# hzxie/RMNet

Measured on AMD Instinct MI355X. Metric: frames/sec at 480p, 1 object, T=5 memory; memory-read HBM GB/s vs peak, higher is better.
Workload: dtype f32 convs; memory read = fp16 operands (K, V, q, P rounded to 11 bits), fp32 accumulate (RMNET_BANK_F16): the frame loop's default for clips with one object -- on one-object 480x854 clips whose masks HAVE a boundary (tests/live_fixture.py) mask IoU vs the CPU path 0.99993-0.99997 and foreground logi

## Files before the change

include/rmnet_hip.h:

```cpp
#ifndef RMNET_HIP_H_
#define RMNET_HIP_H_

#include <stddef.h>
#include <stdint.h>

#ifdef __cplusplus
extern "C" {
#endif

#define RMNET_ABI_VERSION 6

enum {
  RMNET_OK = 0,
  RMNET_E_INVALID_ARG = -1,
  RMNET_E_WORKSPACE = -2,
  RMNET_E_LAUNCH = -3,
  RMNET_E_UNSUPPORTED = -4
};

int rmnet_abi_version(void);
const char *rmnet_error_string(int code);

size_t rmnet_region_map_workspace_bytes(int B, int K, int H, int W);
int rmnet_region_map_f32(const float *mask, int B, int K, int H, int W, float prob_threshold,
// ... 83 lines not shown

#define RMNET_CONV_RELU_IN 1
#define RMNET_CONV_RELU_OUT 2
int rmnet_conv3x3_split_f32(const float *x, const void *wpack, const float *w_unscale, const float *bias, const float *res, int flags,
                            int N, int H, int W, int Cin, float *out, int32_t *range_word, void *stream);

int rmnet_conv3x3_split_lds_f32(const float *x, const void *wpack, const float *w_unscale, const float *bias, const float *res,
                                int flags, int N, int H, int W, int Cin, float *out, int32_t *range_word, void *stream);

int rmnet_conv3x3_rows_f32(const float *x, const void *wpack, const float *w_unscale, const float *bias, const float *res, int flags,
                           int N, int H, int W, int Cin, float *out, int32_t *range_word, void *stream);

int rmnet_conv_split_f32(const float *x, const void *wpack, const float *w_unscale, const float *shift, const float *res, int flags,
                         int N, int H, int W, int Cin, int Cout, int ksize, int stride, float *out, float *out2, int out_split,
                         int32_t *range_word, void *stream);

#define RMNET_CONV_X_SPLIT 4
#define RMNET_CONV_OUT_SPLIT 8
int rmnet_conv_split_pre_f32(const void *x, const void *wpack, const float *w_unscale, const float *shift, const float *res, int flags,
                             int N, int H, int W, int Cin, int Cout, int ksize, int stride, void *out, float *out2, int out_split,
                             int32_t *range_word, void *stream);
int rmnet_split_act_f32(const float *x, long long M, int C, int relu, void *out, int32_t *range_word, void *stream);

int rmnet_conv_rows_pre_f32(const void *x, const void *wpack, const float *w_unscale, const float *shift, const float *res, int flags,
                            int N, int H, int W, int Cin, int Cout, int ksize, int stride, void *out, float *out2, int out_split,
                            int32_t *range_word, void *stream);

int rmnet_stem_split_f32(const float *frame, const float *mask, const float *other, const void *wpack, const float *w_unscale,
                         const float *shift, int N, int H, int W, float *out, int32_t *range_word, void *stream);

int rmnet_flow_stem_f32(const float *img0, const float *img1, long long batch_stride0, long long batch_stride1, const void *wpack,
                        const float *w_unscale, const float *bias, int N, int H, int W, int Hpad, int Wpad, int lh, int lw, float *out, int32_t *range_word, void *stream);

int rmnet_pred_head_f32(const float *x, const float *w, const float *bias, int n, int Hq, int Wq, int C, float *out, void *stream);

#define RMNET_FLOW_RELU 1
#define RMNET_FLOW_LEAKY 2
#define RMNET_FLOW_TRANSPOSED 4
int rmnet_flow_conv_f32(const float *x, int x_ld, const void *wpack, const float *w_unscale, const float *shift, int flags, int N, int H,
                        int W, int Cin, int Cout, int ksize, int stride, float *out, int out_ld, int coff, int32_t *range_word,
                        void *stream);

size_t rmnet_flow_head_workspace_bytes(int N, int H, int W, int Cin);
int rmnet_flow_head_f32(const float *x, int x_ld, const float *wpack, const float *bias, int N, int H, int W, int Cin, float *out,
                        void *workspace, size_t workspace_bytes, void *stream);

// ... 54 lines not shown
```

rmnet_amd/_lib.py:

```python

import ctypes
import os

_HERE = os.path.dirname(os.path.abspath(__file__))
LIB_PATH = os.environ.get('RMNET_HIP_LIB') or os.path.join(_HERE, 'librmnet_hip.so')

c_f32p = ctypes.c_void_p
c_i32p = ctypes.c_void_p
c_f64p = ctypes.POINTER(ctypes.c_double)
c_hostp = ctypes.c_void_p

SIGNATURES = {
    'rmnet_abi_version': (ctypes.c_int, []),
    'rmnet_error_string': (ctypes.c_char_p, [ctypes.c_int]),
    'rmnet_region_map_workspace_bytes': (ctypes.c_size_t, [ctypes.c_int] * 4),
    'rmnet_region_map_f32': (ctypes.c_int, [
        c_f32p, ctypes.c_int, ctypes.c_int, ctypes.c_int, ctypes.c_int, ctypes.c_float, ctypes.c_int,
        ctypes.c_int, c_f32p, c_i32p, c_i32p, ctypes.c_int, ctypes.c_int, ctypes.c_int, ctypes.c_int,
        ctypes.c_int, ctypes.c_void_p, ctypes.c_size_t, ctypes.c_void_p]),
    'rmnet_region_map_warped_f32': (ctypes.c_int, [
        c_f32p, c_f32p, ctypes.c_int, ctypes.c_int, ctypes.c_int, ctypes.c_int, ctypes.c_float, ctypes.c_int,
        ctypes.c_int, c_f32p, c_i32p, c_i32p, ctypes.c_int, ctypes.c_int, ctypes.c_int, ctypes.c_int,
        ctypes.c_int, c_f32p, ctypes.c_void_p, ctypes.c_size_t, ctypes.c_void_p]),
    'rmnet_boxes_to_cell_rects_i32': (ctypes.c_int, [
# ... 53 lines not shown
        c_f32p, c_f32p, c_f32p, c_f32p, c_f32p, c_f32p, ctypes.c_int, ctypes.c_longlong, ctypes.c_int, c_f32p, ctypes.c_void_p]),
    'rmnet_upsample2x_add_nhwc_f32': (ctypes.c_int, [
        c_f32p, c_f32p, ctypes.c_longlong, ctypes.c_int, ctypes.c_int, ctypes.c_int, c_f32p, ctypes.c_void_p]),
    'rmnet_affine_relu_maxpool_nhwc_f32': (ctypes.c_int, [
        c_f32p, c_f32p, c_f32p, ctypes.c_longlong, ctypes.c_int, ctypes.c_int, ctypes.c_int, c_f32p, ctypes.c_void_p]),
    'rmnet_conv3x3_split_f32': (ctypes.c_int, [
        c_f32p, ctypes.c_void_p, c_f32p, c_f32p, c_f32p, ctypes.c_int, ctypes.c_int, ctypes.c_int, ctypes.c_int, ctypes.c_int,
        c_f32p, c_i32p, ctypes.c_void_p]),
    'rmnet_conv3x3_split_lds_f32': (ctypes.c_int, [
        c_f32p, ctypes.c_void_p, c_f32p, c_f32p, c_f32p, ctypes.c_int, ctypes.c_int, ctypes.c_int, ctypes.c_int, ctypes.c_int,
        c_f32p, c_i32p, ctypes.c_void_p]),
    'rmnet_conv3x3_rows_f32': (ctypes.c_int, [
        c_f32p, ctypes.c_void_p, c_f32p, c_f32p, c_f32p, ctypes.c_int, ctypes.c_int, ctypes.c_int, ctypes.c_int, ctypes.c_int,
        c_f32p, c_i32p, ctypes.c_void_p]),
    'rmnet_conv_split_f32': (ctypes.c_int, [
        c_f32p, ctypes.c_void_p, c_f32p, c_f32p, c_f32p, ctypes.c_int, ctypes.c_int, ctypes.c_int, ctypes.c_int, ctypes.c_int,
        ctypes.c_int, ctypes.c_int, ctypes.c_int, c_f32p, c_f32p, ctypes.c_int, c_i32p, ctypes.c_void_p]),
    'rmnet_conv_split_pre_f32': (ctypes.c_int, [
        ctypes.c_void_p, ctypes.c_void_p, c_f32p, c_f32p, c_f32p, ctypes.c_int, ctypes.c_int, ctypes.c_int, ctypes.c_int, ctypes.c_int,
        ctypes.c_int, ctypes.c_int, ctypes.c_int, ctypes.c_void_p, c_f32p, ctypes.c_int, c_i32p, ctypes.c_void_p]),
    'rmnet_conv_rows_pre_f32': (ctypes.c_int, [
        ctypes.c_void_p, ctypes.c_void_p, c_f32p, c_f32p, c_f32p, ctypes.c_int, ctypes.c_int, ctypes.c_int, ctypes.c_int, ctypes.c_int,
        ctypes.c_int, ctypes.c_int, ctypes.c_int, ctypes.c_void_p, c_f32p, ctypes.c_int, c_i32p, ctypes.c_void_p]),
    'rmnet_split_act_f32': (ctypes.c_int, [
        c_f32p, ctypes.c_longlong, ctypes.c_int, ctypes.c_int, ctypes.c_void_p, c_i32p, ctypes.c_void_p]),
    'rmnet_stem_split_f32': (ctypes.c_int, [
        c_f32p, c_f32p, c_f32p, ctypes.c_void_p, c_f32p, c_f32p, ctypes.c_int, ctypes.c_int, ctypes.c_int, c_f32p, c_i32p,
        ctypes.c_void_p]),
    'rmnet_flow_stem_f32': (ctypes.c_int, [
        c_f32p, c_f32p, ctypes.c_longlong, ctypes.c_longlong, ctypes.c_void_p, c_f32p, c_f32p, ctypes.c_int, ctypes.c_int, ctypes.c_int,
        ctypes.c_int, ctypes.c_int, ctypes.c_int, ctypes.c_int, c_f32p, c_i32p, ctypes.c_void_p]),
    'rmnet_pred_head_f32': (ctypes.c_int, [
        c_f32p, c_f32p, c_f32p, ctypes.c_int, ctypes.c_int, ctypes.c_int, ctypes.c_int, c_f32p, ctypes.c_void_p]),
    'rmnet_flow_conv_f32': (ctypes.c_int, [
        c_f32p, ctypes.c_int, ctypes.c_void_p, c_f32p, c_f32p, ctypes.c_int, ctypes.c_int, ctypes.c_int, ctypes.c_int, ctypes.c_int,
        ctypes.c_int, ctypes.c_int, ctypes.c_int, c_f32p, ctypes.c_int, ctypes.c_int, c_i32p, ctypes.c_void_p]),
    'rmnet_flow_head_workspace_bytes': (ctypes.c_size_t, [ctypes.c_int] * 4),
    'rmnet_flow_head_f32': (ctypes.c_int, [
        c_f32p, ctypes.c_int, c_f32p, c_f32p, ctypes.c_int, ctypes.c_int, ctypes.c_int, ctypes.c_int, c_f32p, ctypes.c_void_p,
        ctypes.c_size_t, ctypes.c_void_p]),
    'rmnet_flow_up_f32': (ctypes.c_int, [
        c_f32p, c_f32p, ctypes.c_int, ctypes.c_int, ctypes.c_int, c_f32p, ctypes.c_int, ctypes.c_int, ctypes.c_void_p]),
    'rmnet_flow_affine_f32': (ctypes.c_int, [
        c_f32p, c_f32p, c_f32p, ctypes.c_int, ctypes.c_int, c_f32p, ctypes.c_void_p]),
    'rmnet_flow_affine_workspace_bytes': (ctypes.c_size_t, [ctypes.c_int, ctypes.c_int]),
    'rmnet_flow_affine_f32_host': (ctypes.c_int, [
# ... 72 lines not shown
```

rmnet_amd/csrc/conv_split.hip:

```cpp
#include "split_f16.h"

namespace rmnet {
namespace {

struct SplitArgs {
  const float* x;
  const _Float16* xs;
  const u32x4* wp;
  const float* unscale;
  const float* shift;
  const float* res;
  float* out;
  float* out2;
  _Float16* outs;
  int* range;
  int M, H, W, Ho, Wo, Cin, Cout, csplit, ksize, stride, pad, relu_in, relu_out;
};

template <int WM, int WN, int TI, int TJ, int WPE, bool XS, bool OS>
__global__ __launch_bounds__(kThreads) __attribute__((amdgpu_waves_per_eu(WPE))) void conv_split(SplitArgs a) {
  static_assert(WM * WN * 64 == kThreads, "8 waves");
  constexpr int MT = WM * TI * 16, NT = WN * TJ * 16;
  constexpr int XI = MT / 64;
  constexpr int WI = NT / 64;
  constexpr int kXPlane = MT * kKT, kWPlane = NT * kKT;
  constexpr int kBufHalves = 2 * kXPlane + 2 * kWPlane;
  static_assert(2 * kBufHalves * 2 <= kLdsBytesPerCU, "LDS budget");
  __shared__ __attribute__((aligned(16))) _Float16 lds[2 * kBufHalves];

  const int tid = threadIdx.x, lane = tid & 63, wave = tid >> 6;
  const int wm = wave % WM, wn = wave / WM;
  const int m0 = blockIdx.x * MT, n0 = blockIdx.y * NT;
  const int CB = a.Cin / kKT, steps = a.ksize * a.ksize * CB;
  const int HWo = a.Ho * a.Wo;

  const int c4 = tid & 7;
  int pbase[XI], ph[XI], pw[XI];
#pragma unroll
  for (int i = 0; i < XI; ++i) {
    const int m = m0 + (tid >> 3) + 64 * i;
    const int n = m / HWo, r = m - n * HWo;
    const int ho = r / a.Wo, wo = r - ho * a.Wo;
    ph[i] = m < a.M ? ho * a.stride - a.pad : -4;
    pw[i] = wo * a.stride - a.pad;
    pbase[i] = (n * a.H + ph[i]) * a.W + pw[i];
  }
  f32x4 xr[XI];
  u32x4 xq[XI];
  u32x4 wr[WI];
  int bad = 0;

  auto load_x = [&](int s) {
    const int tap = s / CB, cb = s - tap * CB;
    const int ky = tap / a.ksize, kx = tap - ky * a.ksize;
#pragma unroll
    for (int i = 0; i < XI; ++i) {
      const int h = ph[i] + ky, w = pw[i] + kx;
      const bool in = (unsigned)h < (unsigned)a.H && (unsigned)w < (unsigned)a.W;
      if constexpr (XS) {
        if (in) {
          const unsigned off = (unsigned)(pbase[i] + ky * a.W + kx) * (unsigned)(2 * a.Cin) + (unsigned)(cb * (2 * kKT) + 8 * c4);
          xq[i] = *reinterpret_cast<const u32x4*>(a.xs + off);
        } else {
          xq[i] = u32x4{0u, 0u, 0u, 0u};
        }
      } else {
        if (in) {
          const size_t off = (size_t)(pbase[i] + ky * a.W + kx) * a.Cin + cb * kKT + 4 * c4;
// ... 118 lines not shown
  };
  constexpr bool kInTurn = !XS && TI > TJ && WPE == 4 && WI > 1;
  for (int s = 0; s + 1 < steps; ++s) {
    _Float16* nxt = lds + ((s + 1) & 1) * kBufHalves;
    load_x(s + 1);
    if constexpr (!kInTurn) load_w(s + 1);
    __builtin_amdgcn_sched_barrier(0);
    mma(lds + (s & 1) * kBufHalves, [&] {
      if constexpr (kInTurn) {
        __builtin_amdgcn_sched_barrier(0);
        load_w(s + 1);
        store_x(s + 1, nxt);
        __builtin_amdgcn_sched_barrier(0);
      }
    });
    __builtin_amdgcn_sched_barrier(0);
    if constexpr (!kInTurn) store_x(s + 1, nxt);
    store_w(nxt);
    __syncthreads();
  }
  mma(lds + ((steps - 1) & 1) * kBufHalves, [] {});

  f32x4 r[TI][TJ];
  if (a.res) {
#pragma unroll
    for (int i = 0; i < TI; ++i) {
      const int m = m0 + wm * TI * 16 + i * 16 + fr;
#pragma unroll
      for (int j = 0; j < TJ; ++j) {
        const int co = n0 + wn * TJ * 16 + j * 16 + 4 * fc;
        r[i][j] = m < a.M ? *reinterpret_cast<const f32x4*>(a.res + (size_t)m * a.Cout + co) : f32x4{0.f, 0.f, 0.f, 0.f};
      }
    }
  }
#pragma unroll
  for (int j = 0; j < TJ; ++j) {
    const int co = n0 + wn * TJ * 16 + j * 16 + 4 * fc;
    const f32x4 us = *reinterpret_cast<const f32x4*>(a.unscale + co) * kActUnscale;
    const f32x4 b = a.shift ? *reinterpret_cast<const f32x4*>(a.shift + co) : f32x4{0.f, 0.f, 0.f, 0.f};
#pragma unroll
    for (int i = 0; i < TI; ++i) acc[i][j] = (acc[i][j] + accx[i][j]) * us + b;
  }
#pragma unroll
  for (int j = 0; j < TJ; ++j)
#pragma unroll
    for (int i = 0; i < TI; ++i) asm volatile("" : "+v"(acc[i][j]));
#pragma unroll
  for (int j = 0; j < TJ; ++j) {
    const int co = n0 + wn * TJ * 16 + j * 16 + 4 * fc;
#pragma unroll
    for (int i = 0; i < TI; ++i) {
      const int m = m0 + wm * TI * 16 + i * 16 + fr;
      if (m >= a.M) continue;
      f32x4 v = acc[i][j];
      if (a.res) v += r[i][j];
      if (a.relu_out) {
#pragma unroll
        for (int e = 0; e < 4; ++e) v[e] = v[e] < 0.0f ? 0.0f : v[e];
      }
      if constexpr (OS) {
        half4 hi, lo;
        split4(v, hi, lo, bad);
        _Float16* o = a.outs + (size_t)m * (2 * a.Cout) + (co >> 5) * (2 * kKT) + (co & 31);
        *reinterpret_cast<half4*>(o) = hi;
        *reinterpret_cast<half4*>(o + kKT) = lo;
      } else {
        const size_t off = (size_t)m * a.Cout + co;
        if (!a.out2)
          *reinterpret_cast<f32x4*>(a.out + off) = v;
        else if (co < a.csplit)
          *reinterpret_cast<f32x4*>(a.out + (size_t)m * a.csplit + co) = v;
        else
          *reinterpret_cast<f32x4*>(a.out2 + (size_t)m * (a.Cout - a.csplit) + (co - a.csplit)) = v;
      }
    }
  }
  if (a.range && bad) atomicAdd(a.range, bad);
}

template <int WM, int WN, int TI, int TJ, int WPE, bool XS, bool OS>
void launch(const SplitArgs& a, hipStream_t st) {
  constexpr int MT = WM * TI * 16, NT = WN * TJ * 16;
  hipLaunchKernelGGL((conv_split<WM, WN, TI, TJ, WPE, XS, OS>), dim3((unsigned)((a.M + MT - 1) / MT), (unsigned)(a.Cout / NT)),
                     dim3(kThreads), 0, st, a);
}

template <bool XS, bool OS>
void launch_tile(const SplitArgs& a, hipStream_t st) {
  if (a.Cout % 256 == 0 && (long long)((a.M + 127) / 128) * (a.Cout / 256) >= 512)
    launch<2, 4, 4, 4, 2, XS, OS>(a, st);
  else if (a.Cout % 128 == 0)
    launch<2, 4, 4, 2, 4, XS, OS>(a, st);
  else
    launch<4, 2, 2, 2, 4, XS, OS>(a, st);
}

constexpr int kSplitActThreads = 256;
__global__ __launch_bounds__(kSplitActThreads) void split_act(const float* __restrict__ x, _Float16* __restrict__ out, size_t items,
                                                              int relu, int* range) {
  int bad = 0;
  for (size_t q = (size_t)blockIdx.x * kSplitActThreads + threadIdx.x; q < items; q += (size_t)gridDim.x * kSplitActThreads) {
    f32x4 v[2];
    v[0] = *reinterpret_cast<const f32x4*>(x + q * 8);
// ... 2 lines not shown
#pragma unroll
    for (int k = 0; k < 2; ++k) {
      if (relu) {
#pragma unroll
        for (int e = 0; e < 4; ++e) v[k][e] = v[k][e] < 0.0f ? 0.0f : v[k][e];
      }
      half4 h4, l4;
      split4(v[k], h4, l4, bad);
#pragma unroll
      for (int e = 0; e < 4; ++e) {
        hi[4 * k + e] = h4[e];
        lo[4 * k + e] = l4[e];
      }
    }
    _Float16* o = out + (q >> 2) * (2 * kKT) + (q & 3) * 8;
    *reinterpret_cast<half8*>(o) = hi;
    *reinterpret_cast<half8*>(o + kKT) = lo;
  }
  if (range && bad) atomicAdd(range, bad);
}

int conv_split_entry(const void* x, const void* wpack, const float* w_unscale, const float* shift, const float* res, int flags, int allowed,
                     int N, int H, int W, int Cin, int Cout, int ksize, int stride, void* out, float* out2, int out_split,
                     int32_t* range_word, void* stream) {
  if (!x || !wpack || !w_unscale || !out || N <= 0 || H <= 0 || W <= 0 || Cin <= 0 || Cout <= 0) return RMNET_E_INVALID_ARG;
  if (flags & ~allowed) return RMNET_E_INVALID_ARG;
  const bool xs = (flags & RMNET_CONV_X_SPLIT) != 0, os = (flags & RMNET_CONV_OUT_SPLIT) != 0;
  if (xs && (flags & RMNET_CONV_RELU_IN)) return RMNET_E_INVALID_ARG;
  if (os && out2) return RMNET_E_INVALID_ARG;
  if ((reinterpret_cast<uintptr_t>(x) | reinterpret_cast<uintptr_t>(wpack) | reinterpret_cast<uintptr_t>(w_unscale) |
       reinterpret_cast<uintptr_t>(shift) | reinterpret_cast<uintptr_t>(res) | reinterpret_cast<uintptr_t>(out) |
       reinterpret_cast<uintptr_t>(out2)) & 15)
    return RMNET_E_INVALID_ARG;
  if (out2 && (res || out_split <= 0 || out_split >= Cout || out_split % 4)) return RMNET_E_INVALID_ARG;
  if ((ksize != 1 && ksize != 3) || (stride != 1 && stride != 2)) return RMNET_E_UNSUPPORTED;
  if (Cin % kKT || Cout % 64) return RMNET_E_UNSUPPORTED;
  const int pad = ksize / 2;
  const int Ho = (H + 2 * pad - ksize) / stride + 1, Wo = (W + 2 * pad - ksize) / stride + 1;
  const long long Mi = (long long)N * H * W, M = (long long)N * Ho * Wo;
  if (Mi * Cin >= (1LL << 31) || M * Cout >= (1LL << 31)) return RMNET_E_UNSUPPORTED;
  const long long xbytes = Mi * Cin * 4, c1 = out2 ? out_split : Cout;
  if (overlap(out, M * c1 * 4, x, xbytes)) return RMNET_E_INVALID_ARG;
  if (os && res && overlap(out, M * c1 * 4, res, M * Cout * 4)) return RMNET_E_INVALID_ARG;
  if (out2) {
    if (overlap(out2, M * (Cout - c1) * 4, x, xbytes) || overlap(out2, M * (Cout - c1) * 4, out, M * c1 * 4)) return RMNET_E_INVALID_ARG;
  }
  SplitArgs a;
  a.x = xs ? nullptr : reinterpret_cast<const float*>(x);
  a.xs = xs ? reinterpret_cast<const _Float16*>(x) : nullptr;
  a.wp = reinterpret_cast<const u32x4*>(wpack); a.unscale = w_unscale; a.shift = shift; a.res = res;
  a.out = os ? nullptr : reinterpret_cast<float*>(out); a.out2 = out2; a.outs = os ? reinterpret_cast<_Float16*>(out) : nullptr;
  a.range = range_word; a.M = (int)M; a.H = H; a.W = W; a.Ho = Ho; a.Wo = Wo; a.Cin = Cin; a.Cout = Cout; a.csplit = (int)c1;
  a.ksize = ksize; a.stride = stride; a.pad = pad;
  a.relu_in = (flags & RMNET_CONV_RELU_IN) != 0;
  a.relu_out = (flags & RMNET_CONV_RELU_OUT) != 0;
  hipStream_t st = (hipStream_t)stream;
  if (xs && os) launch_tile<true, true>(a, st);
  else if (xs) launch_tile<true, false>(a, st);
  else if (os) launch_tile<false, true>(a, st);
  else launch_tile<false, false>(a, st);
  return check_launch();
}

}
}

extern "C" int rmnet_conv_split_f32(const float* x, const void* wpack, const float* w_unscale, const float* shift,
                                    const float* res, int flags, int N, int H, int W, int Cin, int Cout, int ksize, int stride,
                                    float* out, float* out2, int out_split, int32_t* range_word, void* stream) {
  return rmnet::conv_split_entry(x, wpack, w_unscale, shift, res, flags, RMNET_CONV_RELU_IN | RMNET_CONV_RELU_OUT, N, H, W, Cin, Cout,
                                 ksize, stride, out, out2, out_split, range_word, stream);
}

extern "C" int rmnet_conv_split_pre_f32(const void* x, const void* wpack, const float* w_unscale, const float* shift, const float* res,
                                        int flags, int N, int H, int W, int Cin, int Cout, int ksize, int stride, void* out, float* out2,
                                        int out_split, int32_t* range_word, void* stream) {
  return rmnet::conv_split_entry(x, wpack, w_unscale, shift, res, flags,
                                 RMNET_CONV_RELU_IN | RMNET_CONV_RELU_OUT | RMNET_CONV_X_SPLIT | RMNET_CONV_OUT_SPLIT, N, H, W, Cin, Cout,
                                 ksize, stride, out, out2, out_split, range_word, stream);
}

extern "C" int rmnet_split_act_f32(const float* x, long long M, int C, int relu, void* out, int32_t* range_word, void* stream) {
  using namespace rmnet;
  if (!x || !out || M <= 0 || C <= 0) return RMNET_E_INVALID_ARG;
  if ((reinterpret_cast<uintptr_t>(x) | reinterpret_cast<uintptr_t>(out)) & 15) return RMNET_E_INVALID_ARG;
  if (C % kKT) return RMNET_E_UNSUPPORTED;
  if (M > (1LL << 40) / C) return RMNET_E_UNSUPPORTED;
  if (overlap(out, M * C * 4, x, M * C * 4)) return RMNET_E_INVALID_ARG;
  const size_t items = (size_t)M * C / 8;
  const size_t blocks = (items + kSplitActThreads - 1) / kSplitActThreads;
  const unsigned grid = (unsigned)(blocks < (size_t)kNumCUs * 8 ? blocks : (size_t)kNumCUs * 8);
  hipLaunchKernelGGL(split_act, dim3(grid), dim3(kSplitActThreads), 0, (hipStream_t)stream, x, reinterpret_cast<_Float16*>(out), items,
                     relu != 0, range_word);
  return check_launch();
}
```

rmnet_amd/networks.py:

```python

import torch
import torch.nn.functional as F
from torch import nn


class _Bottleneck(nn.Module):

    def __init__(self, c_in, width, stride, project):
        super().__init__()
        c_out = width * 4
        self.conv1 = nn.Conv2d(c_in, width, 1, bias=False)
        self.bn1 = nn.BatchNorm2d(width)
        self.conv2 = nn.Conv2d(width, width, 3, stride=stride, padding=1, bias=False)
        self.bn2 = nn.BatchNorm2d(width)
        self.conv3 = nn.Conv2d(width, c_out, 1, bias=False)
        self.bn3 = nn.BatchNorm2d(c_out)
        self.relu = nn.ReLU(inplace=True)
        self.downsample = None
        if project:
            self.downsample = nn.Sequential(nn.Conv2d(c_in, c_out, 1, stride=stride, bias=False),
                                            nn.BatchNorm2d(c_out))

    def forward(self, x):
        if getattr(self, '_fused', False) and not self.training and x.is_cuda:
# ... 258 lines not shown


def set_split_conv_(module, enable):
    prev = {}
    for m in module.modules():
        if isinstance(m, (_Bottleneck, KeyValue, ResBlock, Refine, Decoder, EncoderMemory, EncoderQuery)):
            prev[m] = getattr(m, '_conv_split', False)
            m._conv_split = bool(enable) and getattr(m, '_wu', getattr(m, '_wu1', None)) is not None
    return prev


def restore_split_conv_(prev):
    for m, v in prev.items():
        m._conv_split = v


class KeyValue(nn.Module):

    def __init__(self, indim, keydim, valdim):
        super().__init__()
        self.key_conv = nn.Conv2d(indim, keydim, 3, padding=1)
        self.value_conv = nn.Conv2d(indim, valdim, 3, padding=1)

    def forward(self, x):
        if _split_path_ok(self, x, self.key_conv, ('full', 'split', 'trunk')):
            from . import ops
            x = x.contiguous(memory_format=torch.channels_last)
            rw = ops.conv_range_word(x.device)
            if conv_presplit():
                x = ops.split_act(x, range_word=rw)
            return ops.conv_split(x, self._wp, self._wu, self._bkv, ksize=3, range_word=rw, split=self.key_conv.out_channels)
        return self.key_conv(x), self.value_conv(x)


def _hash_uniform(n, seed):
    m32 = 0xFFFFFFFF
    x = (torch.arange(n, dtype=torch.int64) * 2654435761 + seed * 40503 + 0x9E3779B9) & m32
    x = x ^ (x >> 16)
    x = (x * 0x85EBCA6B) & m32
    x = x ^ (x >> 13)
    x = (x * 0xC2B2AE35) & m32
    x = x ^ (x >> 16)
    return x.to(torch.float64) * (2.0 / 4294967296.0) - 1.0


def procedural_init_(module, gain=0.9):
    import math
    with torch.no_grad():
        for name, t in module.state_dict().items():
            if name.endswith('num_batches_tracked'):
                continue
            seed = sum((i + 1) * ord(ch) for i, ch in enumerate(name)) % 1000003
            n = t.numel()
# ... 167 lines not shown
```

rmnet_amd/ops.py:

```python

import ctypes
import os

import numpy as np
import torch

from . import _lib


MR_FORCE_GENERIC = 1
MR_EXACT_FP32 = 2
BANK_MAX_SLOTS = 2048


def _check(t, name, dtype=torch.float32):
    if not isinstance(t, torch.Tensor):
        raise RuntimeError('%s must be a torch.Tensor' % name)
    if not t.is_cuda:
        raise RuntimeError('%s must be a CUDA tensor' % name)
    if not t.is_contiguous():
        raise RuntimeError('%s must be contiguous' % name)
    if t.dtype != dtype:
        raise RuntimeError('%s must be %s, got %s' % (name, dtype, t.dtype))

# ... 655 lines not shown
    out = torch.empty((N, H, W, C // 32, 2, 32), dtype=torch.float16, device=x.device)
    lib = _lib.load()
    with torch.cuda.device(x.device):
        rc = lib.rmnet_split_act_f32(_ptr(x), N * H * W, C, 1 if relu else 0, _ptr(out), _ptr(range_word), _stream(x.device))
    _lib.check(rc, 'rmnet_split_act_f32')
    return out


TRUNK_ROWS_DEFAULT = True
TRUNK_ROWS_ENTRY = 'rmnet_conv_rows_pre_f32'
TRUNK_ROWS_ALL = (64, 128, 256)
TRUNK_ROWS_CLASSES = (128, 256)


def trunk_rows_enabled():
    v = os.environ.get('RMNET_TRUNK_ROWS')
    if v is None:
        return TRUNK_ROWS_DEFAULT
    if v.strip() not in ('0', '1'):
        raise RuntimeError("RMNET_TRUNK_ROWS must be '0' or '1', got %r" % v)
    return v.strip() == '1'


def conv_split(x, wpack, w_unscale, shift=None, res=None, ksize=3, stride=1, relu_in=False, relu_out=False, out=None,
               range_word=None, split=None, out_presplit=False):
    x_split = is_split_act(x)
    if x_split:
        _check_split_act(x, 'x')
        N, H, W = x.shape[:3]
        cin = x.shape[3] * 32
        if relu_in:
            raise RuntimeError('conv_split: relu_in cannot be applied to a split activation (its producer applies it)')
    else:
        _check_act(x, 'x')
        if x.dim() != 4 or not x.is_contiguous(memory_format=torch.channels_last):
            raise RuntimeError('x must be a channels-last [N, Cin, H, W] tensor')
        N, cin, H, W = x.shape
    if ksize not in (1, 3) or stride not in (1, 2):
        raise RuntimeError('conv_split implements ksize 1 / 3 and stride 1 / 2, got %r / %r' % (ksize, stride))
    _check(w_unscale, 'w_unscale')
    cout = w_unscale.numel()
    if cin % 32 or cout % 64 or cout == 0:
        raise RuntimeError('conv_split needs Cin % 32 == 0 and Cout % 64 == 0, got %d, %d' % (cin, cout))
    _check(wpack, 'wpack', torch.int16)
    if wpack.numel() != ksize * ksize * cin * cout * 2:
        raise RuntimeError('wpack has %d elements, a %dx%d Cin = %d Cout = %d pack has %d'
                           % (wpack.numel(), ksize, ksize, cin, cout, ksize * ksize * cin * cout * 2))
    pad = ksize // 2
    shape = (N, cout, (H + 2 * pad - ksize) // stride + 1, (W + 2 * pad - ksize) // stride + 1)
    if shift is not None:
        _check(shift, 'shift')
        if shift.numel() != cout:
            raise RuntimeError('shift must have Cout = %d elements' % cout)
    if res is not None:
        _check_act(res, 'res')
        if tuple(res.shape) != shape or not res.is_contiguous(memory_format=torch.channels_last):
            raise RuntimeError('res must be a channels-last %s tensor' % (shape,))
    out2 = None
    if out_presplit:
        if split is not None or out is not None:
            raise RuntimeError('conv_split: out_presplit returns one new split activation, without split / out')
        out = torch.empty((N, shape[2], shape[3], cout // 32, 2, 32), dtype=torch.float16, device=x.device)
    elif split is not None:
        if res is not None or out is not None or not 0 < split < cout or split % 4:
            raise RuntimeError('conv_split: split must be a multiple of 4 in (0, %d), without res / out' % cout)
        out = torch.empty((N, split) + shape[2:], dtype=torch.float32, device=x.device, memory_format=torch.channels_last)
        out2 = torch.empty((N, cout - split) + shape[2:], dtype=torch.float32, device=x.device, memory_format=torch.channels_last)
    elif out is None:
        out = torch.empty(shape, dtype=torch.float32, device=x.device, memory_format=torch.channels_last)
    else:
        _check_act(out, 'out')
        if tuple(out.shape) != shape or not out.is_contiguous(memory_format=torch.channels_last):
            raise RuntimeError('out must be a channels-last %s tensor' % (shape,))
    if range_word is not None:
        _check(range_word, 'range_word', torch.int32)
    for t in (wpack, w_unscale, shift, res, out, range_word):
        if t is not None and t.device != x.device:
            raise RuntimeError('conv_split: every tensor must be on %s' % x.device)
    flags = (CONV_RELU_IN if relu_in else 0) | (CONV_RELU_OUT if relu_out else 0)
    rows = trunk_rows_enabled() and x_split and ksize == 3 and stride == 1 and cin == cout and cin in TRUNK_ROWS_CLASSES \
        and res is None and split is None
    lib = _lib.load()
    with torch.cuda.device(x.device):
        if x_split or out_presplit:
            flags |= (CONV_X_SPLIT if x_split else 0) | (CONV_OUT_SPLIT if out_presplit else 0)
            what = TRUNK_ROWS_ENTRY if rows else 'rmnet_conv_split_pre_f32'
            rc = getattr(lib, what)(_ptr(x), _ptr(wpack), _ptr(w_unscale), _ptr(shift), _ptr(res), flags, N, H, W, cin,
                                    cout, ksize, stride, _ptr(out), _ptr(out2), split or 0, _ptr(range_word),
                                    _stream(x.device))
        else:
            what = 'rmnet_conv_split_f32'
            rc = lib.rmnet_conv_split_f32(_ptr(x), _ptr(wpack), _ptr(w_unscale), _ptr(shift), _ptr(res), flags, N, H, W, cin, cout,
                                          ksize, stride, _ptr(out), _ptr(out2), split or 0, _ptr(range_word), _stream(x.device))
    _lib.check(rc, what)
    return out if out2 is None else (out, out2)


FLOW_RELU, FLOW_LEAKY, FLOW_TRANSPOSED = 1, 2, 4
_FLOW_ACT = {None: 0, False: 0, 'none': 0, True: FLOW_RELU, 'relu': FLOW_RELU, 'leaky': FLOW_LEAKY}


def flow_conv_phase_weights(weight):
# ... 666 lines not shown
```

rmnet_amd/rmnet.py:

```python

import torch
import torch.nn.functional as F
from torch import nn

from . import ops
from .helpers import pad_amounts, pad_divide_by
from .networks import Decoder, EncoderMemory, EncoderQuery, KeyValue, Refine, ResBlock
from .reg_att_map_generator import RegionalAttentionMapGenerator

_ABSENT_LOGIT = -16.1181
_NEW_OBJECT_SCALE = 32.0605


class MemoryReader(nn.Module):

    def __init__(self, return_affinity=False, precision='split'):
        super().__init__()
        self.return_affinity = return_affinity
        self.precision = ops._precision(precision)

    def forward(self, m_key, m_val, q_key, q_val, mem_rects=None, qry_rects=None, T=None):
        return ops.memory_read(m_key.contiguous(), m_val.contiguous(), q_key.contiguous(),
                               q_val.contiguous(), mem_rects, qry_rects,
                               want_p=self.return_affinity, T=T,
# ... 91 lines not shown
                at += n_objects[b]
            out.append(padded)
        return out

    def warp(self, img0, flow):
        B, C, H, W = img0.shape
        vgrid = self._base_grid(B, H, W, img0.device) + flow
        gx = 2.0 * vgrid[:, 0] / max(W - 1, 1) - 1.0
        gy = 2.0 * vgrid[:, 1] / max(H - 1, 1) - 1.0
        grid = torch.stack((gx, gy), dim=3)
        img1 = F.grid_sample(img0, grid, align_corners=True)
        mask = F.grid_sample(torch.ones_like(img0), grid, align_corners=True)
        mask = (mask >= 0.9999).to(img0.dtype)
        return img1 * mask, mask

    def get_att_map(self, prev_mask, flow=None):
        expt = prev_mask if flow is None else self.warp(prev_mask, flow)[0]
        return self.att_map_generator(expt.contiguous())

    def _inference_only(self):
        if self.training:
            raise RuntimeError('rmnet_amd.RMNet is inference-only (its HIP kernels have no autograd): call .eval()')

    def _encode_memory(self, frame, masks, n_objects):
        B, K, H, W = masks.shape
        (frame, masks), _ = pad_divide_by([frame, masks.float()], 16, (H, W))
        if all(int(n) == 1 for n in n_objects):
            f_in, m_in = frame, masks[:, 1]
            o_in = None
        else:
            fs, ms, os_ = [], [], []
            for b in range(B):
                n = n_objects[b]
                for o in range(1, n + 1):
                    fs.append(frame[b:b + 1])
                    ms.append(masks[b, o:o + 1])
                    if n == 1:
                        os_.append(torch.zeros_like(masks[b, o:o + 1]))
                    else:
                        others = masks[b, 1:o].sum(0, keepdim=True) + masks[b, o + 1:n + 1].sum(0, keepdim=True)
                        os_.append(others.clamp(0, 1))
            f_in, m_in, o_in = torch.cat(fs), torch.cat(ms), torch.cat(os_)
        r4 = self.encoder_memory(f_in, m_in, o_in)[0]
        k4, v4 = self.kv_memory(r4)
        h, w = k4.shape[-2:]
        _, bboxes, rects = ops.region_map(masks.contiguous(), want_map=False, cell_grid=(0, 0, 16, h, w))
        return k4, v4, bboxes, rects

    @torch.no_grad()
    def memorize(self, frame, masks, n_objects):
        self._inference_only()
        B, K = masks.shape[:2]
        k4, v4, bboxes, rects = self._encode_memory(frame, masks, n_objects)
        k4, v4 = self.pad_memory([k4, v4], n_objects, K)
        r = rects.view(B * K, 1, 4)
        k4 = ops.rect_mask(k4.view(B * K, -1, 1, *k4.shape[-2:]).contiguous(), r).view_as(k4)
        v4 = ops.rect_mask(v4.view(B * K, -1, 1, *v4.shape[-2:]).contiguous(), r).view_as(v4)
        return k4, v4, bboxes

    def soft_aggregation(self, ps, K, n_objects):
        B = len(n_objects)
        em = ps.new_zeros(B, K, *ps.shape[1:])
        at = 0
        for b in range(B):
            sl = ps[at:at + n_objects[b]]
            em[b, 0] = torch.prod(1 - sl, dim=0)
            em[b, 1:n_objects[b] + 1] = sl
            at += n_objects[b]
        em = torch.clamp(em, 1e-7, 1 - 1e-7)
        return torch.log(em / (1 - em))

    def _segment_core(self, frame, qry_rects, m_key, m_val, mem_rects, T, n_objects, K, batch_of_obj,
                      obj_begin=None):
        (frame,), pad = pad_divide_by([frame], 16, frame.shape[2:])
        r4, r3, r2, _, _ = self.encoder_query(frame)
        k4, v4 = self.kv_query(r4)
        if all(int(n) == 1 for n in n_objects):
            k4e, v4e, r3e, r2e = k4, v4, r3, r2
        else:
            k4e, v4e = k4.index_select(0, batch_of_obj), v4.index_select(0, batch_of_obj)
            r3e, r2e = r3.index_select(0, batch_of_obj), r2.index_select(0, batch_of_obj)
        ev = getattr(self, '_profile_events', None)
        if isinstance(m_key, (ops.MemoryBank, ops.TensorBank)):
            if T is None:
                m4 = m_key.read_staged(k4e.contiguous(), v4e.contiguous(), qry_rects, events=ev)
            else:
                m4 = m_key.read(T, k4e.contiguous(), v4e.contiguous(), qry_rects, events=ev)
        else:
            m4, _ = ops.memory_read(m_key, m_val, k4e.contiguous(), v4e.contiguous(), mem_rects, qry_rects,
                                    T=T, events=ev)
        if obj_begin is not None and (getattr(self, '_fused_tail', False) and not self.training):
            return ops.soft_aggregate(self.decoder(m4, r3e, r2e).contiguous(), obj_begin, K, pad, want_prob=True)
        ps = F.softmax(self.decoder(m4, r3e, r2e), dim=1)[:, 1]
        logit = self.soft_aggregation(ps, K, n_objects)
        lw, uw, lh, uh = pad
        return logit[:, :, lh:logit.shape[2] - uh, lw:logit.shape[3] - uw]

    @torch.no_grad()
    def segment(self, frame, att_map, keys, values, prev_bboxes, curr_bbox, n_objects):
# ... 19 lines not shown
            self.lw, self.lh = lw, lh
            self.h, self.w = (H + lh + uh) // 16, (W + lw + uw) // 16
            self.device = device
            begin = [0]
            for n in self.n_max:
                begin.append(begin[-1] + n)
            self.obj_begin = torch.tensor(begin, dtype=torch.int32, device=device)

    def new_bank(self, ctx, capacity, exact=False, precision=None):
        if exact:
            return ops.TensorBank(len(ctx.flat), capacity, ctx.h, ctx.w, ctx.device)
        return ops.MemoryBank(len(ctx.flat), capacity, ctx.h, ctx.w, ctx.device,
                              precision=precision or self.resolve_read_precision(ctx.n_max))

    def resolve_read_precision(self, n_objects):
        if self.read_precision != 'auto':
            return self.read_precision
        return 'f16' if not getattr(self, '_auto_peaked', False) and all(int(n) <= 1 for n in n_objects) else 'split'

    @torch.no_grad()
    def frame_step(self, ctx, bank, prev_frame, prev_mask, cur_frame, cur_flow, commit):
        self._inference_only()
        B, K = ctx.B, ctx.K
        k4, v4, boxes, rects = self._encode_memory(prev_frame, prev_mask, ctx.n_max)
        bank.stage(k4.contiguous(), v4.contiguous(), rects.view(B * K, 4).index_select(0, ctx.flat))
        if getattr(self, '_fused_tail', False) and self._fused_warp_ok(prev_mask.device):
            _, _, q_rects = ops.region_map(prev_mask.contiguous(), want_map=False, flow=cur_flow.contiguous(),
                                           cell_grid=(ctx.lw, ctx.lh, 16, ctx.h, ctx.w))
        else:
            expt = self.warp(prev_mask, cur_flow)[0]
            _, _, q_rects = ops.region_map(expt.contiguous(), want_map=False,
                                           cell_grid=(ctx.lw, ctx.lh, 16, ctx.h, ctx.w))
        q_rects = q_rects.view(B * K, 4).index_select(0, ctx.flat)
        out = self._segment_core(cur_frame, q_rects, bank, None, None, None, ctx.n_max, K, ctx.batch_of_obj,
                                 obj_begin=ctx.obj_begin)
        if commit:
            bank.commit()
        return out

    @torch.no_grad()
    def forward(self, frames, masks, optical_flows, n_objects, memorize_every, device=None, _exact=False, graph=None,
                return_logits=False, _precision=None, object_plan=None):
        self._inference_only()
        dev = torch.device('cuda', torch.cuda.current_device()) if device is None else torch.device(device)
        frames = frames.to(dev, non_blocking=True)
        optical_flows = optical_flows.to(dev, non_blocking=True)
        plans, sampling = None, None
        if object_plan is not None:
            if len(object_plan) == 3:
                labels_dev, plans, sampling = object_plan
            else:
                labels_dev, plans = object_plan
            masks = masks[:, :1]
        masks_dev = masks.to(dev, non_blocking=True)
        B, N, _, H, W = frames.shape
        K = masks.shape[2]
        est = torch.zeros(B, N, K, H, W, device=dev)
        est[:, 0] = masks_dev[:, 0]
# ... 142 lines not shown
```

Before: 668.3.

## Compute key/value convs only inside each object's region rectangle

Adds a regional variant of the split-activation key/value 3x3 conv. It computes output cells only inside each object's rectangle and zero-fills the cells outside, with a prefix-sum over rect areas mapping GEMM rows to cells. The memory encoder now computes region rects before encoding and passes them to kv_memory. For single-object clips, the query KV conv uses the query rects. This cuts conv FLOPs on frames where objects cover a small area, at the cost of binary-search indexing, a scatter-style NCHW store and an extra zero-fill pass. It relies on downstream memory reads ignoring values outside the rects.

```diff
diff --git a/include/rmnet_hip.h b/include/rmnet_hip.h
--- a/include/rmnet_hip.h
+++ b/include/rmnet_hip.h
@@ -129,6 +129,10 @@
                              int32_t *range_word, void *stream);
 int rmnet_split_act_f32(const float *x, long long M, int C, int relu, void *out, int32_t *range_word, void *stream);
 
+int rmnet_conv_split_region_f32(const void *x, const void *wpack, const float *w_unscale, const float *shift, int flags, int N, int H,
+                                int W, int Cin, int Cout, int ksize, int stride, const int32_t *rects, float *out, float *out2,
+                                int out_split, int32_t *range_word, void *stream);
+
 int rmnet_conv_rows_pre_f32(const void *x, const void *wpack, const float *w_unscale, const float *shift, const float *res, int flags,
                             int N, int H, int W, int Cin, int Cout, int ksize, int stride, void *out, float *out2, int out_split,
                             int32_t *range_word, void *stream);
diff --git a/rmnet_amd/_lib.py b/rmnet_amd/_lib.py
--- a/rmnet_amd/_lib.py
+++ b/rmnet_amd/_lib.py
@@ -99,6 +99,9 @@
     'rmnet_conv_rows_pre_f32': (ctypes.c_int, [
         ctypes.c_void_p, ctypes.c_void_p, c_f32p, c_f32p, c_f32p, ctypes.c_int, ctypes.c_int, ctypes.c_int, ctypes.c_int, ctypes.c_int,
         ctypes.c_int, ctypes.c_int, ctypes.c_int, ctypes.c_void_p, c_f32p, ctypes.c_int, c_i32p, ctypes.c_void_p]),
+    'rmnet_conv_split_region_f32': (ctypes.c_int, [
+        ctypes.c_void_p, ctypes.c_void_p, c_f32p, c_f32p, ctypes.c_int, ctypes.c_int, ctypes.c_int, ctypes.c_int, ctypes.c_int,
+        ctypes.c_int, ctypes.c_int, ctypes.c_int, c_i32p, c_f32p, c_f32p, ctypes.c_int, c_i32p, ctypes.c_void_p]),
     'rmnet_split_act_f32': (ctypes.c_int, [
         c_f32p, ctypes.c_longlong, ctypes.c_int, ctypes.c_int, ctypes.c_void_p, c_i32p, ctypes.c_void_p]),
     'rmnet_stem_split_f32': (ctypes.c_int, [
diff --git a/rmnet_amd/csrc/conv_split.hip b/rmnet_amd/csrc/conv_split.hip
--- a/rmnet_amd/csrc/conv_split.hip
+++ b/rmnet_amd/csrc/conv_split.hip
@@ -17,9 +17,35 @@
   int M, H, W, Ho, Wo, Cin, Cout, csplit, ksize, stride, pad, relu_in, relu_out;
 };
 
-template <int WM, int WN, int TI, int TJ, int WPE, bool XS, bool OS>
-__global__ __launch_bounds__(kThreads) __attribute__((amdgpu_waves_per_eu(WPE))) void conv_split(SplitArgs a) {
+struct RegionArgs : SplitArgs {
+  const int32_t* rects;
+};
+constexpr int kRegionMaxObjects = 64;
+
+struct RegionTables {
+  int pref[kRegionMaxObjects + 1];
+  int rect[kRegionMaxObjects][4];
+};
+__device__ __forceinline__ RegionTables& region_tables() {
+  __shared__ RegionTables t;
+  return t;
+}
+__device__ __forceinline__ void region_row(const RegionTables& t, int NO, int g, int& o, int& cy, int& cx) {
+  int lo = 0, hi = NO;
+  while (hi - lo > 1) {
+    const int mid = (lo + hi) >> 1;
+    if (t.pref[mid] <= g) lo = mid; else hi = mid;
+  }
+  const int n = g - t.pref[lo], rw = t.rect[lo][1] - t.rect[lo][0] + 1, ry = n / rw;
+  o = lo;
+  cy = t.rect[lo][2] + ry;
+  cx = t.rect[lo][0] + (n - ry * rw);
+}
+
+template <int WM, int WN, int TI, int TJ, int WPE, bool XS, bool OS, bool RG, class Args>
+__device__ __forceinline__ void conv_split_body(const Args a) {
   static_assert(WM * WN * 64 == kThreads, "8 waves");
+  static_assert(!RG || (XS && !OS), "the regional instance takes a split input and writes fp32");
   constexpr int MT = WM * TI * 16, NT = WN * TJ * 16;
   constexpr int XI = MT / 64;
   constexpr int WI = NT / 64;
@@ -36,14 +62,63 @@
 
   const int c4 = tid & 7;
   int pbase[XI], ph[XI], pw[XI];
-#pragma unroll
-  for (int i = 0; i < XI; ++i) {
-    const int m = m0 + (tid >> 3) + 64 * i;
-    const int n = m / HWo, r = m - n * HWo;
-    const int ho = r / a.Wo, wo = r - ho * a.Wo;
-    ph[i] = m < a.M ? ho * a.stride - a.pad : -4;
-    pw[i] = wo * a.stride - a.pad;
-    pbase[i] = (n * a.H + ph[i]) * a.W + pw[i];
+  if constexpr (RG) {
+    RegionTables& rt = region_tables();
+    const int NO = a.M / HWo;
+    if (tid < RMNET_WAVE) {
+      Rect rc{1, 0, 1, 0};
+      if (tid < NO) {
+        const int32_t* r = a.rects + 4 * tid;
+        rc = Rect{max(r[0], 0), min(r[1], a.W - 1), max(r[2], 0), min(r[3], a.H - 1)};
+      }
+      const int incl = wave_scan_incl_fast(rc.area());
+      if (tid == 0) rt.pref[0] = 0;
+      if (tid < NO) {
+        rt.pref[tid + 1] = incl;
+        rt.rect[tid][0] = rc.cx0; rt.rect[tid][1] = rc.cx1; rt.rect[tid][2] = rc.cy0; rt.rect[tid][3] = rc.cy1;
+      }
+    }
+    __syncthreads();
+    {
+      static_assert(kThreads % MT == 0, "a thread of the fill owns one cell");
+      const int f = m0 + tid % MT;
+      bool fill = f < a.M;
+      const int o = fill ? f / HWo : 0, cell = f - o * HWo;
+      if (fill) {
+        const int cy = cell / a.Wo, cx = cell - cy * a.Wo;
+        fill = !Rect{rt.rect[o][0], rt.rect[o][1], rt.rect[o][2], rt.rect[o][3]}.contains(cy, cx);
+      }
+      if (fill) {
+        const int c2 = a.Cout - a.csplit;
+        for (int c = n0 + tid / MT; c < n0 + NT; c += kThreads / MT) {
+          if (c < a.csplit)
+            a.out[((size_t)o * a.csplit + c) * HWo + cell] = 0.0f;
+          else
+            a.out2[((size_t)o * c2 + (c - a.csplit)) * HWo + cell] = 0.0f;
+        }
+      }
+    }
+    const int total = rt.pref[NO];
+    if (m0 >= total) return;
+#pragma unroll
+    for (int i = 0; i < XI; ++i) {
+      const int g = m0 + (tid >> 3) + 64 * i;
+      int o = 0, cy = -4 + a.pad, cx = a.pad;
+      if (g < total) region_row(rt, NO, g, o, cy, cx);
+      ph[i] = cy - a.pad;
+      pw[i] = cx - a.pad;
+      pbase[i] = (o * a.H + ph[i]) * a.W + pw[i];
+    }
+  } else {
+#pragma unroll
+    for (int i = 0; i < XI; ++i) {
+      const int m = m0 + (tid >> 3) + 64 * i;
+      const int n = m / HWo, r = m - n * HWo;
+      const int ho = r / a.Wo, wo = r - ho * a.Wo;
+      ph[i] = m < a.M ? ho * a.stride - a.pad : -4;
+      pw[i] = wo * a.stride - a.pad;
+      pbase[i] = (n * a.H + ph[i]) * a.W + pw[i];
+    }
   }
   f32x4 xr[XI];
   u32x4 xq[XI];
@@ -208,7 +283,7 @@
   mma(lds + ((steps - 1) & 1) * kBufHalves, [] {});
 
   f32x4 r[TI][TJ];
-  if (a.res) {
+  if (!RG && a.res) {
 #pragma unroll
     for (int i = 0; i < TI; ++i) {
       const int m = m0 + wm * TI * 16 + i * 16 + fr;
@@ -231,6 +306,39 @@
   for (int j = 0; j < TJ; ++j)
 #pragma unroll
     for (int i = 0; i < TI; ++i) asm volatile("" : "+v"(acc[i][j]));
+  if constexpr (RG) {
+    const RegionTables& rt = region_tables();
+    const int NO = a.M / HWo, total = rt.pref[NO];
+    int po[TI], pcell[TI];
+#pragma unroll
+    for (int i = 0; i < TI; ++i) {
+      const int g = m0 + wm * TI * 16 + i * 16 + fr;
+      int cy = 0, cx = 0;
+      po[i] = -1;
+      if (g < total) region_row(rt, NO, g, po[i], cy, cx);
+      pcell[i] = cy * a.Wo + cx;
+    }
+    const int c2 = a.Cout - a.csplit;
+#pragma unroll
+    for (int j = 0; j < TJ; ++j) {
+      const int co = n0 + wn * TJ * 16 + j * 16 + 4 * fc;
+      const bool key = co < a.csplit;
+#pragma unroll
+      for (int i = 0; i < TI; ++i) {
+        if (po[i] < 0) continue;
+        f32x4 v = acc[i][j];
+        if (a.relu_out) {
+#pragma unroll
+          for (int e = 0; e < 4; ++e) v[e] = v[e] < 0.0f ? 0.0f : v[e];
+        }
+        float* o = key ? a.out + ((size_t)po[i] * a.csplit + co) * HWo + pcell[i]
+                       : a.out2 + ((size_t)po[i] * c2 + (co - a.csplit)) * HWo + pcell[i];
+#pragma unroll
+        for (int e = 0; e < 4; ++e) o[(size_t)e * HWo] = v[e];
+      }
+    }
+    return;
+  }
 #pragma unroll
   for (int j = 0; j < TJ; ++j) {
     const int co = n0 + wn * TJ * 16 + j * 16 + 4 * fc;
@@ -265,6 +373,15 @@
 }
 
 template <int WM, int WN, int TI, int TJ, int WPE, bool XS, bool OS>
+__global__ __launch_bounds__(kThreads) __attribute__((amdgpu_waves_per_eu(WPE))) void conv_split(SplitArgs a) {
+  conv_split_body<WM, WN, TI, TJ, WPE, XS, OS, false>(a);
+}
+
+__global__ __launch_bounds__(kThreads) __attribute__((amdgpu_waves_per_eu(4))) void conv_split_region(RegionArgs a) {
+  conv_split_body<2, 4, 4, 2, 4, true, false, true>(a);
+}
+
+template <int WM, int WN, int TI, int TJ, int WPE, bool XS, bool OS>
 void launch(const SplitArgs& a, hipStream_t st) {
   constexpr int MT = WM * TI * 16, NT = WN * TJ * 16;
   hipLaunchKernelGGL((conv_split<WM, WN, TI, TJ, WPE, XS, OS>), dim3((unsigned)((a.M + MT - 1) / MT), (unsigned)(a.Cout / NT)),
@@ -313,12 +430,13 @@
 
 int conv_split_entry(const void* x, const void* wpack, const float* w_unscale, const float* shift, const float* res, int flags, int allowed,
                      int N, int H, int W, int Cin, int Cout, int ksize, int stride, void* out, float* out2, int out_split,
-                     int32_t* range_word, void* stream) {
+                     int32_t* range_word, void* stream, bool region = false, const int32_t* rects = nullptr) {
   if (!x || !wpack || !w_unscale || !out || N <= 0 || H <= 0 || W <= 0 || Cin <= 0 || Cout <= 0) return RMNET_E_INVALID_ARG;
   if (flags & ~allowed) return RMNET_E_INVALID_ARG;
   const bool xs = (flags & RMNET_CONV_X_SPLIT) != 0, os = (flags & RMNET_CONV_OUT_SPLIT) != 0;
   if (xs && (flags & RMNET_CONV_RELU_IN)) return RMNET_E_INVALID_ARG;
   if (os && out2) return RMNET_E_INVALID_ARG;
+  if (region && (!rects || !xs || !out2 || (reinterpret_cast<uintptr_t>(rects) & 15))) return RMNET_E_INVALID_ARG;
   if ((reinterpret_cast<uintptr_t>(x) | reinterpret_cast<uintptr_t>(wpack) | reinterpret_cast<uintptr_t>(w_unscale) |
        reinterpret_cast<uintptr_t>(shift) | reinterpret_cast<uintptr_t>(res) | reinterpret_cast<uintptr_t>(out) |
        reinterpret_cast<uintptr_t>(out2)) & 15)
@@ -326,6 +444,7 @@
   if (out2 && (res || out_split <= 0 || out_split >= Cout || out_split % 4)) return RMNET_E_INVALID_ARG;
   if ((ksize != 1 && ksize != 3) || (stride != 1 && stride != 2)) return RMNET_E_UNSUPPORTED;
   if (Cin % kKT || Cout % 64) return RMNET_E_UNSUPPORTED;
+  if (region && (ksize != 3 || stride != 1 || Cout % 128 || N > kRegionMaxObjects)) return RMNET_E_UNSUPPORTED;
   const int pad = ksize / 2;
   const int Ho = (H + 2 * pad - ksize) / stride + 1, Wo = (W + 2 * pad - ksize) / stride + 1;
   const long long Mi = (long long)N * H * W, M = (long long)N * Ho * Wo;
@@ -336,7 +455,9 @@
   if (out2) {
     if (overlap(out2, M * (Cout - c1) * 4, x, xbytes) || overlap(out2, M * (Cout - c1) * 4, out, M * c1 * 4)) return RMNET_E_INVALID_ARG;
   }
-  SplitArgs a;
+  if (region && (overlap(out, M * c1 * 4, rects, 16LL * N) || overlap(out2, M * (Cout - c1) * 4, rects, 16LL * N))) return RMNET_E_INVALID_ARG;
+  RegionArgs a;
+  a.rects = rects;
   a.x = xs ? nullptr : reinterpret_cast<const float*>(x);
   a.xs = xs ? reinterpret_cast<const _Float16*>(x) : nullptr;
   a.wp = reinterpret_cast<const u32x4*>(wpack); a.unscale = w_unscale; a.shift = shift; a.res = res;
@@ -346,7 +467,9 @@
   a.relu_in = (flags & RMNET_CONV_RELU_IN) != 0;
   a.relu_out = (flags & RMNET_CONV_RELU_OUT) != 0;
   hipStream_t st = (hipStream_t)stream;
-  if (xs && os) launch_tile<true, true>(a, st);
+  if (region)
+    hipLaunchKernelGGL(conv_split_region, dim3((unsigned)((a.M + 127) / 128), (unsigned)(a.Cout / 128)), dim3(kThreads), 0, st, a);
+  else if (xs && os) launch_tile<true, true>(a, st);
   else if (xs) launch_tile<true, false>(a, st);
   else if (os) launch_tile<false, true>(a, st);
   else launch_tile<false, false>(a, st);
@@ -369,6 +492,13 @@
   return rmnet::conv_split_entry(x, wpack, w_unscale, shift, res, flags,
                                  RMNET_CONV_RELU_IN | RMNET_CONV_RELU_OUT | RMNET_CONV_X_SPLIT | RMNET_CONV_OUT_SPLIT, N, H, W, Cin, Cout,
                                  ksize, stride, out, out2, out_split, range_word, stream);
+}
+
+extern "C" int rmnet_conv_split_region_f32(const void* x, const void* wpack, const float* w_unscale, const float* shift, int flags, int N,
+                                           int H, int W, int Cin, int Cout, int ksize, int stride, const int32_t* rects, float* out,
+                                           float* out2, int out_split, int32_t* range_word, void* stream) {
+  return rmnet::conv_split_entry(x, wpack, w_unscale, shift, nullptr, flags, RMNET_CONV_RELU_OUT | RMNET_CONV_X_SPLIT, N, H, W, Cin, Cout,
+                                 ksize, stride, out, out2, out_split, range_word, stream, true, rects);
 }
 
 extern "C" int rmnet_split_act_f32(const float* x, long long M, int C, int relu, void* out, int32_t* range_word, void* stream) {
diff --git a/rmnet_amd/networks.py b/rmnet_amd/networks.py
--- a/rmnet_amd/networks.py
+++ b/rmnet_amd/networks.py
@@ -304,13 +304,16 @@
         self.key_conv = nn.Conv2d(indim, keydim, 3, padding=1)
         self.value_conv = nn.Conv2d(indim, valdim, 3, padding=1)
 
-    def forward(self, x):
+    def forward(self, x, rects=None):
         if _split_path_ok(self, x, self.key_conv, ('full', 'split', 'trunk')):
             from . import ops
             x = x.contiguous(memory_format=torch.channels_last)
             rw = ops.conv_range_word(x.device)
             if conv_presplit():
                 x = ops.split_act(x, range_word=rw)
+                if rects is not None and x.shape[0] <= ops.KV_REGION_MAX_OBJECTS:
+                    return ops.conv_split(x, self._wp, self._wu, self._bkv, ksize=3, range_word=rw, split=self.key_conv.out_channels,
+                                          rects=rects)
             return ops.conv_split(x, self._wp, self._wu, self._bkv, ksize=3, range_word=rw, split=self.key_conv.out_channels)
         return self.key_conv(x), self.value_conv(x)
 
diff --git a/rmnet_amd/ops.py b/rmnet_amd/ops.py
--- a/rmnet_amd/ops.py
+++ b/rmnet_amd/ops.py
@@ -701,8 +701,22 @@
     return v.strip() == '1'
 
 
+KV_REGION_DEFAULT = True
+KV_REGION_ENTRY = 'rmnet_conv_split_region_f32'
+KV_REGION_MAX_OBJECTS = 64
+
+
+def kv_region_enabled():
+    v = os.environ.get('RMNET_KV_REGION')
+    if v is None:
+        return KV_REGION_DEFAULT
+    if v.strip() not in ('0', '1'):
+        raise RuntimeError("RMNET_KV_REGION must be '0' or '1', got %r" % v)
+    return v.strip() == '1'
+
+
 def conv_split(x, wpack, w_unscale, shift=None, res=None, ksize=3, stride=1, relu_in=False, relu_out=False, out=None,
-               range_word=None, split=None, out_presplit=False):
+               range_word=None, split=None, out_presplit=False, rects=None, _out=None):
     x_split = is_split_act(x)
     if x_split:
         _check_split_act(x, 'x')
@@ -736,7 +750,26 @@
         if tuple(res.shape) != shape or not res.is_contiguous(memory_format=torch.channels_last):
             raise RuntimeError('res must be a channels-last %s tensor' % (shape,))
     out2 = None
-    if out_presplit:
+    if rects is not None:
+        if not x_split or ksize != 3 or stride != 1 or split is None or res is not None or out is not None or out_presplit \
+                or relu_in or cout % 128 or not 0 < split < cout or split % 4:
+            raise RuntimeError('conv_split: rects needs a split-activation x, ksize 3, stride 1, split= (a multiple of 4 in (0, Cout)) '
+                               'and Cout % 128 == 0, without res / out / out_presplit')
+        _check(rects, 'rects', torch.int32)
+        if tuple(rects.shape) != (N, 4):
+            raise RuntimeError('rects must be [N, 4] = %s, got %s' % ((N, 4), tuple(rects.shape)))
+        if _out is None:
+            out = torch.empty((N, split) + shape[2:], dtype=torch.float32, device=x.device)
+            out2 = torch.empty((N, cout - split) + shape[2:], dtype=torch.float32, device=x.device)
+        else:
+            out, out2 = _out
+            for t, c in ((out, split), (out2, cout - split)):
+                _check(t, '_out')
+                if tuple(t.shape) != (N, c) + shape[2:]:
+                    raise RuntimeError('_out must be the NCHW pair %s / %s' % ((N, split) + shape[2:], (N, cout - split) + shape[2:]))
+    elif _out is not None:
+        raise RuntimeError('conv_split: _out goes with rects')
+    elif out_presplit:
         if split is not None or out is not None:
             raise RuntimeError('conv_split: out_presplit returns one new split activation, without split / out')
         out = torch.empty((N, shape[2], shape[3], cout // 32, 2, 32), dtype=torch.float16, device=x.device)
@@ -753,10 +786,17 @@
             raise RuntimeError('out must be a channels-last %s tensor' % (shape,))
     if range_word is not None:
         _check(range_word, 'range_word', torch.int32)
-    for t in (wpack, w_unscale, shift, res, out, range_word):
+    for t in (wpack, w_unscale, shift, res, out, out2, range_word, rects):
         if t is not None and t.device != x.device:
             raise RuntimeError('conv_split: every tensor must be on %s' % x.device)
     flags = (CONV_RELU_IN if relu_in else 0) | (CONV_RELU_OUT if relu_out else 0)
+    if rects is not None:
+        with torch.cuda.device(x.device):
+            rc = _lib.load().rmnet_conv_split_region_f32(_ptr(x), _ptr(wpack), _ptr(w_unscale), _ptr(shift), flags | CONV_X_SPLIT, N, H, W,
+                                                         cin, cout, ksize, stride, _ptr(rects), _ptr(out), _ptr(out2), split,
+                                                         _ptr(range_word), _stream(x.device))
+        _lib.check(rc, KV_REGION_ENTRY)
+        return out, out2
     rows = trunk_rows_enabled() and x_split and ksize == 3 and stride == 1 and cin == cout and cin in TRUNK_ROWS_CLASSES \
         and res is None and split is None
     lib = _lib.load()
diff --git a/rmnet_amd/rmnet.py b/rmnet_amd/rmnet.py
--- a/rmnet_amd/rmnet.py
+++ b/rmnet_amd/rmnet.py
@@ -137,9 +137,11 @@
         if self.training:
             raise RuntimeError('rmnet_amd.RMNet is inference-only (its HIP kernels have no autograd): call .eval()')
 
-    def _encode_memory(self, frame, masks, n_objects):
+    def _encode_memory(self, frame, masks, n_objects, regional=False, flat=None):
         B, K, H, W = masks.shape
         (frame, masks), _ = pad_divide_by([frame, masks.float()], 16, (H, W))
+        _, bboxes, rects = ops.region_map(masks.contiguous(), want_map=False,
+                                          cell_grid=(0, 0, 16, masks.shape[2] // 16, masks.shape[3] // 16))
         if all(int(n) == 1 for n in n_objects):
             f_in, m_in = frame, masks[:, 1]
             o_in = None
@@ -157,9 +159,11 @@
                         os_.append(others.clamp(0, 1))
             f_in, m_in, o_in = torch.cat(fs), torch.cat(ms), torch.cat(os_)
         r4 = self.encoder_memory(f_in, m_in, o_in)[0]
+        if regional:
+            obj_rects = rects.view(B * K, 4).index_select(0, flat)
+            k4, v4 = self.kv_memory(r4, obj_rects)
+            return k4, v4, bboxes, rects, obj_rects
         k4, v4 = self.kv_memory(r4)
-        h, w = k4.shape[-2:]
-        _, bboxes, rects = ops.region_map(masks.contiguous(), want_map=False, cell_grid=(0, 0, 16, h, w))
         return k4, v4, bboxes, rects
 
     @torch.no_grad()
@@ -186,10 +190,10 @@
         return torch.log(em / (1 - em))
 
     def _segment_core(self, frame, qry_rects, m_key, m_val, mem_rects, T, n_objects, K, batch_of_obj,
-                      obj_begin=None):
+                      obj_begin=None, kv_rects=None):
         (frame,), pad = pad_divide_by([frame], 16, frame.shape[2:])
         r4, r3, r2, _, _ = self.encoder_query(frame)
-        k4, v4 = self.kv_query(r4)
+        k4, v4 = self.kv_query(r4, kv_rects)
         if all(int(n) == 1 for n in n_objects):
             k4e, v4e, r3e, r2e = k4, v4, r3, r2
         else:
@@ -255,8 +259,13 @@
     def frame_step(self, ctx, bank, prev_frame, prev_mask, cur_frame, cur_flow, commit):
         self._inference_only()
         B, K = ctx.B, ctx.K
-        k4, v4, boxes, rects = self._encode_memory(prev_frame, prev_mask, ctx.n_max)
-        bank.stage(k4.contiguous(), v4.contiguous(), rects.view(B * K, 4).index_select(0, ctx.flat))
+        regional = ops.kv_region_enabled() and isinstance(bank, ops.MemoryBank)
+        if regional:
+            k4, v4, boxes, rects, obj_rects = self._encode_memory(prev_frame, prev_mask, ctx.n_max, regional=True, flat=ctx.flat)
+        else:
+            k4, v4, boxes, rects = self._encode_memory(prev_frame, prev_mask, ctx.n_max)
+            obj_rects = rects.view(B * K, 4).index_select(0, ctx.flat)
+        bank.stage(k4.contiguous(), v4.contiguous(), obj_rects)
         if getattr(self, '_fused_tail', False) and self._fused_warp_ok(prev_mask.device):
             _, _, q_rects = ops.region_map(prev_mask.contiguous(), want_map=False, flow=cur_flow.contiguous(),
                                            cell_grid=(ctx.lw, ctx.lh, 16, ctx.h, ctx.w))
@@ -266,7 +275,8 @@
                                            cell_grid=(ctx.lw, ctx.lh, 16, ctx.h, ctx.w))
         q_rects = q_rects.view(B * K, 4).index_select(0, ctx.flat)
         out = self._segment_core(cur_frame, q_rects, bank, None, None, None, ctx.n_max, K, ctx.batch_of_obj,
-                                 obj_begin=ctx.obj_begin)
+                                 obj_begin=ctx.obj_begin,
+                                 kv_rects=q_rects if regional and all(int(n) == 1 for n in ctx.n_max) else None)
         if commit:
             bank.commit()
         return out
```

After: 698.2, median of 6. 1.04x the previous value.
